# dsforza96/yocto-hair

Measured on AMD Instinct MI355X. Metric: Msamples/sec (whole node), 720x720x1536spp sphere-hairblock; per-pixel L2 vs CPU ref, higher is better.
Workload: dtype f32

## Files before the change

### include/yhair.h

```cpp
#ifndef YHAIR_H_
#define YHAIR_H_

#include <stdint.h>

#ifdef __cplusplus
extern "C" {
#endif

#define YH_OK 0
#define YH_E_INVALID -1
#define YH_E_DEVICE -2
#define YH_E_STATE -3
#define YH_E_IO -4
#define YH_E_SELFTEST -5


typedef struct yh_shape {
  int          num_vertices;
  const float* positions;
  const float* normals;
  const float* radius;
  int          num_lines;
  const int*   lines;
  int          num_triangles;
// ... 296 lines not shown
int yh_bvh_build_wide(int n, const float* boxes, int width, float* slots);

int yh_bvh_build_gpu(yh_context* ctx, int n, const float* boxes, float* nodes, int* primitives);
int yh_bvh_build_wide_gpu(yh_context* ctx, int n, const float* boxes, int width, float* slots);
int yh_bvh_refit_wide(int n, const float* boxes, const int* primitives, int width, float* slots);
int yh_bvh_refit_wide_gpu(yh_context* ctx, int n, const float* boxes, const int* primitives, int width, float* slots);

int yh_surface_lobe_batch(yh_context* ctx, int kind, int n, const float* params,
    const float* normal, const float* outgoing, const float* incoming,
    const float* rn, float* out);
int yh_surface_bsdf_batch(yh_context* ctx, int n, const yh_material* materials,
    const float* normal, const float* outgoing, const float* incoming,
    const float* rn, float* out);
int yh_intersect_batch(yh_context* ctx, int n, const float* rays, int* object,
    int* element, float* uv, float* distance);
#define YH_INTERSECT_FORMS 7
#define YH_INTERSECT_TABLE_IN_MEMORY 16
int yh_intersect_plain_batch(yh_context* ctx, int form, int n, const float* rays,
    int* object, int* element, float* uv, float* distance);
int yh_intersect_plain_form(int form);
int yh_scene_once(const yh_context* ctx);
int yh_lights_const_env(const yh_context* ctx);
int yh_shade_regions(const yh_context* ctx, uint64_t* out, int capacity);

int yh_lights_batch(yh_context* ctx, int form, int n, const float* position,
    const float* direction, const float* rn, float* out);

#define YH_VOLUME_FLOATS 24
int yh_volume_batch(yh_context* ctx, int form, int tex, int n,
    const yh_material* materials, const float* normal, const float* outgoing,
    const float* incoming, const float* texval, const float* rn, float* out);
#define YH_POINT_POSITION        0
#define YH_POINT_NORMAL          3
#define YH_POINT_SHADING_NORMAL  6
#define YH_POINT_TEXCOORD        9
#define YH_POINT_COLOR_TEX      11
#define YH_POINT_EMISSION_TEX   14
#define YH_POINT_EMISSION_TEX_X 17
#define YH_POINT_SCATTERING_TEX 18
#define YH_POINT_EMISSION       21
#define YH_POINT_BSDF           24
#define YH_POINT_DENSITY        46
#define YH_POINT_SCATTER        49
#define YH_POINT_ANISOTROPY     52
#define YH_POINT_FLOATS         53
int yh_point_batch(yh_context* ctx, int form, int n, const int* object,
// ... 34 lines not shown
```

### yocto-hair_amd/csrc/dev_items.h

```cpp
#ifndef YH_DEV_ITEMS_H_
#define YH_DEV_ITEMS_H_
#include "dev_path.h"

using namespace yhd;

#define YH_BLOCK 512
#define YH_MIN_WAVES 4

#define YH_QUADS (YH_BLOCK / 4)
template <bool COUNT, bool GENERAL, int BLOCK, int SHADER, int MODE = YH_MODE_QUAD, bool ONCE = false, bool TRIM = false, bool CENV = false>
YH_DEV void trace_items(const yhd_scene& sc, const yhd_state& st, int nsamples, yhd_counters* counters, unsigned int block = blockIdx.x,
    unsigned int blocks = gridDim.x) {
  constexpr int LPP    = YH_IS_HEX(MODE) ? 16 : YH_IS_OCT(MODE) ? 8 : 4;
  constexpr int GROUPS = BLOCK / LPP;
  extern __shared__ v4f lds_dyn[];
  YH_LDS unsigned int* lds_stack = (YH_LDS unsigned int*)lds_dyn;
  YH_LDS v4f*          lds_tabs  = (YH_LDS v4f*)(lds_stack + ((MODE == YH_MODE_QUAD ? sc.stack_entries : YH_IS_HEX(MODE) ? sc.stack_entries16 : sc.stack_entries8) + YH_HITROWS) * GROUPS);
  trace_ctx tc;
  tc.sc = &sc;
  tc.ls = nullptr, tc.sc_dev = nullptr;
  YH_LDS float* lds_cam;
  stage_tables(sc, lds_tabs, threadIdx.x, blockDim.x, tc, lds_cam);
  __syncthreads();

// ... 73 lines not shown
      }
      if (COUNT) {
        c1 = clock64(), cyc_trace += c1 - c0;
        unsigned int smax = steps;
        for (int off = 32; off > 0; off >>= 1) smax = max(smax, (unsigned int)__shfl_xor((int)smax, off, 64));
        w_steps += smax, l_steps += (lane & 3) == 0 ? steps : 0;
      }
      YH_REGION_MARK("shade_head");
      if (alive) {
        if constexpr (CENV) alive = path_step<COUNT, GROUPS, GENERAL, TRIM, CENV>(tc, ps, isec, rng, st.bounces, &ce);
        else if constexpr (SHADER == YH_SHADER_PATH) alive = path_step<COUNT, GROUPS, GENERAL, TRIM>(tc, ps, isec, rng, st.bounces);
        else alive = shade_step<COUNT, GROUPS, SHADER>(tc, ps, isec, rng, st.bounces);
        if (!alive) {
          YH_REGION_MARK("end");
          if (COUNT) stats.from = clock64();
          path_end(ps, st.clamp, acc);
          if (COUNT) count_quad<COUNT>(stats.samples);
          count_region<COUNT>(tc.stats, YH_REGION_END, stats.from);
        }
      }
      YH_REGION_MARK("loop_tail");
      if (COUNT) cyc_shade += clock64() - c1;
    }
    if (COUNT) {
      unsigned int v[11] = {stats.samples, stats.rays, stats.nodes, stats.seg, stats.tri, stats.hair, stats.surf,
          stats.envl, stats.envs, l_steps, l_iters};
      for (int k = 0; k < 11; k++)
        for (int off = 32; off > 0; off >>= 1) v[k] += (unsigned int)__shfl_xor((int)v[k], off, 64);
      if (lane == 0) {
        atomicAdd(&counters->samples, (unsigned long long)v[0]), atomicAdd(&counters->rays, (unsigned long long)v[1]);
        atomicAdd(&counters->nodes, (unsigned long long)v[2]), atomicAdd(&counters->seg, (unsigned long long)v[3]);
        atomicAdd(&counters->tri, (unsigned long long)v[4]), atomicAdd(&counters->hair, (unsigned long long)v[5]);
        atomicAdd(&counters->surf, (unsigned long long)v[6]), atomicAdd(&counters->envl, (unsigned long long)v[7]);
        atomicAdd(&counters->envs, (unsigned long long)v[8]);
        atomicAdd(&counters->lane_steps, (unsigned long long)v[9]), atomicAdd(&counters->lane_iters, (unsigned long long)v[10]);
        atomicAdd(&counters->cyc_trace, cyc_trace), atomicAdd(&counters->cyc_shade, cyc_shade);
        atomicAdd(&counters->wave_iters, (unsigned long long)w_iters), atomicAdd(&counters->wave_steps, (unsigned long long)w_steps);
      }
      if (lane == 0) {
        atomicAdd(&counters->c_geom, stats.c_geom), atomicAdd(&counters->c_sample, stats.c_sample);
        atomicAdd(&counters->c_eval, stats.c_eval), atomicAdd(&counters->c_rest, stats.c_rest);
      }
      {
        unsigned int b[10] = {stats.t_node, stats.l_node, stats.t_line, stats.l_line, stats.t_tri, stats.l_tri, stats.t_enter,
            stats.l_enter, stats.t_scene, stats.l_scene};
        for (int k = 0; k < 10; k++) {
          for (int off = 32; off > 0; off >>= 1) b[k] += (unsigned int)__shfl_xor((int)b[k], off, 64);
          if (lane == 0) atomicAdd(&counters->branch[k], (unsigned long long)b[k]);
        }
      }
      unsigned long long* sums = stats.r;
      if (lane < 3 * YH_REGIONS) atomicAdd(&counters->region[lane], sums[lane]), sums[lane] = 0;
      stats = stats_t{};
      stats.r = sums;
    }
    if (owner && (lane & (LPP - 1)) == 0) {
      st.rng_state[pix] = rng.state;
      st.accum[pix]     = acc;
    }
    if (lane == 0) {
      unsigned int dt = (unsigned int)(wall_clock64() - t0);
      if (YH_IS_OCT(MODE) || YH_IS_HEX(MODE)) atomicAdd(&st.tile_cost[item], dt);
      else st.tile_cost[item] = dt;
      if (COUNT) atomicAdd(&counters->cyc_tile, (unsigned long long)dt);
    }
  }
}
#define YH_OCT_BLOCK 256
template <bool COUNT, bool GENERAL, int BLOCK, int WAVES, int MODE = YH_MODE_QUAD, bool ONCE = false>
__global__ __launch_bounds__(BLOCK, WAVES) void k_trace(const yhd_scene sc, const yhd_state st,
    int nsamples, yhd_counters* counters) {
  static_assert(!ONCE || !GENERAL, "the prologue form exists for the plain variants");
  constexpr bool TRIM = !GENERAL && BLOCK == YH_BLOCK && MODE == YH_MODE_QUAD;
  trace_items<COUNT, GENERAL, BLOCK, YH_SHADER_PATH, MODE, ONCE, TRIM>(sc, st, nsamples, counters);
}
template <bool COUNT, bool ONCE>
__global__ __launch_bounds__(YH_BLOCK, YH_MIN_WAVES) void k_trace_cenv(const yhd_scene sc, const yhd_state st, int nsamples, yhd_counters* counters) {
  trace_items<COUNT, false, YH_BLOCK, YH_SHADER_PATH, YH_MODE_QUAD, ONCE, true, true>(sc, st, nsamples, counters);
}
template <bool GENERAL, bool ONCE = false>
__global__ __launch_bounds__(YH_BLOCK, YH_MIN_WAVES) void k_trace_sbs(const yhd_scene sc, const yhd_state st, int nsamples, int oct_blocks,
    int quad_items, int oct_entries) {
  if ((int)blockIdx.x < oct_blocks) {
    yhd_state so   = st;
    so.tiles       = st.tiles + quad_items, so.num_tiles = oct_entries, so.tile_cursor = st.tile_cursor + 16;
    trace_items<false, GENERAL, YH_BLOCK, YH_SHADER_PATH, YH_MODE_OCT, ONCE, !GENERAL>(sc, so, nsamples, nullptr, blockIdx.x, (unsigned)oct_blocks);
  } else {
// ... 20 lines not shown
```

### yocto-hair_amd/csrc/dev_trace.h

```cpp
#ifndef YH_DEV_TRACE_H_
#define YH_DEV_TRACE_H_
#include "dev_math.h"

namespace yhd {

struct rng_t {
  uint64_t state, inc;
};
YH_DEV uint32_t advance_rng(rng_t& rng) {
  uint64_t old        = rng.state;
  rng.state           = old * 6364136223846793005ULL + rng.inc;
  uint32_t xorshifted = (uint32_t)(((old >> 18u) ^ old) >> 27u);
  uint32_t rot        = (uint32_t)(old >> 59u);
  return (xorshifted >> rot) | (xorshifted << ((-rot) & 31));
}
YH_DEV float rand1f(rng_t& rng) {
  return __uint_as_float((advance_rng(rng) >> 9) | 0x3f800000u) - 1.0f;
}
YH_DEV rng_t make_rng(uint64_t seed, uint64_t seq) {
  rng_t rng;
  rng.state = 0U;
  rng.inc   = (seq << 1u) | 1u;
  advance_rng(rng);
  rng.state += seed;
  advance_rng(rng);
  return rng;
}

struct ray_t {
  f3    o, d;
  float tmin, tmax;
};
YH_DEV ray_t mkray(f3 o, f3 d) { return ray_t{o, d, ray_eps, flt_max}; }

struct hit_t {
  int   object, slot;
  float u, v, distance;
};

template <bool STRAIGHT = false, bool RAW = false>
YH_DEV bool intersect_line(f3 ro, f3 rd, float tmin, float tmax, f3 p0, f3 p1, float r0,
    float r1, float& uu, float& vv, float& dist, float a_in = 0.0f, float* rr = nullptr) {
  f3    u = rd, v = p1 - p0, w = ro - p0;
  float a = RAW ? a_in : dot(u, u), b = dot(u, v), c = dot(v, v), d = dot(u, w), e = dot(v, w);
  float det = a * c - b * b;
  if (STRAIGHT) {
    float t   = (b * e - c * d) / det;
    float s   = (a * e - b * d) / det;
    bool  ok  = det != 0 && !(t < tmin || t > tmax);
    s         = fclamp(s, 0.0f, 1.0f);
    f3    pr  = ro + rd * t;
    f3    pl  = p0 + (p1 - p0) * s;
    f3    prl = pr - pl;
    float d2  = dot(prl, prl);
    float r   = r0 * (1 - s) + r1 * s;
    ok        = ok && !(d2 > r * r);
    if (RAW) {
      uu = s, vv = d2, *rr = r, dist = t;
      return ok;
    }
    if (ok) uu = s, vv = sqrtf(d2) / r, dist = t;
    return ok;
  }
  if (det == 0) return false;
  float t = (b * e - c * d) / det;
  float s = (a * e - b * d) / det;
  if (t < tmin || t > tmax) return false;
  s        = fclamp(s, 0.0f, 1.0f);
// ... 6 lines not shown
  if (RAW) uu = s, vv = d2, *rr = r;
  else uu = s, vv = sqrtf(d2) / r;
  dist = t;
  return true;
}
YH_DEV bool intersect_triangle(f3 ro, f3 rd, float tmin, float tmax, f3 p0, f3 p1, f3 p2,
    float& uu, float& vv, float& dist) {
  f3    edge1 = p1 - p0, edge2 = p2 - p0;
  f3    pvec = cross(rd, edge2);
  float det  = dot(edge1, pvec);
  if (det == 0) return false;
  float inv_det = 1.0f / det;
  f3    tvec    = ro - p0;
  float u       = dot(tvec, pvec) * inv_det;
  if (u < 0 || u > 1) return false;
  f3    qvec = cross(tvec, edge1);
  float v    = dot(rd, qvec) * inv_det;
  if (v < 0 || u + v > 1) return false;
  float t = dot(edge2, qvec) * inv_det;
  if (t < tmin || t > tmax) return false;
  uu = u, vv = v;
  dist = t;
  return true;
}
YH_DEV bool intersect_bbox(f3 ro, f3 dinv, float tmin_, float tmax_, f3 bmin, f3 bmax) {
  f3    it_min = (bmin - ro) * dinv;
  f3    it_max = (bmax - ro) * dinv;
  f3    tmin   = {fmin_(it_min.x, it_max.x), fmin_(it_min.y, it_max.y), fmin_(it_min.z, it_max.z)};
  f3    tmax   = {fmax_(it_min.x, it_max.x), fmax_(it_min.y, it_max.y), fmax_(it_min.z, it_max.z)};
  float t0     = fmax_(hmax(tmin), tmin_);
  float t1     = fmin_(hmin(tmax), tmax_);
  t1 *= 1.00000024f;
  return t0 <= t1;
}

YH_DEV bool intersect_bbox_nonan(f3 ro, f3 dinv, float tmin_, float tmax_, f3 bmin, f3 bmax) {
  f3    it_min = (bmin - ro) * dinv;
  f3    it_max = (bmax - ro) * dinv;
  float t0 = __builtin_fmaxf(__builtin_fmaxf(__builtin_fminf(it_min.x, it_max.x), __builtin_fminf(it_min.y, it_max.y)),
      __builtin_fmaxf(__builtin_fminf(it_min.z, it_max.z), tmin_));
  float t1 = __builtin_fminf(__builtin_fminf(__builtin_fmaxf(it_min.x, it_max.x), __builtin_fmaxf(it_min.y, it_max.y)),
      __builtin_fminf(__builtin_fmaxf(it_min.z, it_max.z), tmax_));
  t1 *= 1.00000024f;
  return t0 <= t1;
}

// ... 139 lines not shown
  auto box_test = [](f3 o, f3 dinv, float t0, float t1, f3 bmin, f3 bmax) {
    return EXACT ? intersect_bbox(o, dinv, t0, t1, bmin, bmax) : intersect_bbox_nonan(o, dinv, t0, t1, bmin, bmax);
  };
  if (!EXACT && !wnonan) {
    redo = true;
    return hit;
  }
  f3    lo = ray.o, ld = ray.d, ldinv = wdinv;
  constexpr bool HOIST_A = STRIDE != 64;
  float ld2 = 0.0f;
  int   lsign = wsign | (wsign << 4), cur_obj = -1, kind = 0, node_base = 0;
  unsigned long long n_nodes = 0, n_seg = 0, n_tri = 0;
  unsigned int       n_steps = 0;

  const bool in_lds = LDS_SCENE || tc.lds_scene != nullptr;
  const bool wide_scene = !LDS_SCENE && sc.scene_wide_root >= 0;
  const YH_LDS v4f* lds_snodes = in_lds ? tc.lds_scene + YH_OBJECT_F4 * sc.num_objects : nullptr;
  auto scene_prim = [&](int i) -> int {
    if (in_lds) return ((const YH_LDS int*)(lds_snodes + 2 * sc.num_scene_nodes))[i];
    return sc.scene_prims[i];
  };
  static_assert(!ONCE || (LDS_SCENE && !EXACT), "the prologue form reads the scene level from LDS and leaves NaN slabs to the second pass");
  unsigned int cur;
  if constexpr (ONCE) {
    cur = YH_NONE;
    const v4f n0 = lds_snodes[0], n1 = lds_snodes[1];
    if (q == 0) n_nodes++;
    if (COUNT) count_branch<COUNT>(tc.stats->t_scene, tc.stats->l_scene);
    if (COUNT) count_branch<COUNT>(tc.stats->t_enter, tc.stats->l_enter);
    if (box_test(ray.o, wdinv, ray.tmin, tmax, xyz(n0), xyz(n1))) {
      const int start = __float_as_int(n0.w), num = __float_as_int(n1.w) & 0xffff;
      for (int k = num - 1; k >= 0; k--) {
        const int         obj = scene_prim(start + k);
        const YH_LDS v4f* ob  = tc.lds_scene + YH_OBJECT_F4 * obj;
        const f3    it_min = (xyz(ob[8]) - ray.o) * wdinv, it_max = (xyz(ob[9]) - ray.o) * wdinv;
        const float t0  = __builtin_fmaxf(__builtin_fmaxf(__builtin_fminf(it_min.x, it_max.x), __builtin_fminf(it_min.y, it_max.y)),
            __builtin_fmaxf(__builtin_fminf(it_min.z, it_max.z), ray.tmin));
        const float far = __builtin_fminf(__builtin_fminf(__builtin_fmaxf(it_min.x, it_max.x), __builtin_fmaxf(it_min.y, it_max.y)),
            __builtin_fmaxf(it_min.z, it_max.z));
        if (!(t0 <= __builtin_fminf(far, tmax) * 1.00000024f)) continue;
        const v4f a = ob[3], b = ob[4], c = ob[5];
        frame     inv;
        inv.x = {a.x, a.y, a.z}, inv.y = {a.w, b.x, b.y}, inv.z = {b.z, b.w, c.x}, inv.o = {c.y, c.z, c.w};
        const f3  o_ = transform_point(inv, ray.o), d_ = transform_vector(inv, ray.d), di = quad_rcp(d_);
        const int sg = (di.x < 0 ? 1 : 0) | (di.y < 0 ? 2 : 0) | (di.z < 0 ? 4 : 0);
        if (!(finite3(di) && finite3(o_))) redo = true;
        const int root = __float_as_int(YH_IS_HEX(MODE) ? ob[10].w : YH_IS_OCT(MODE) ? ob[10].z : ob[10].x);
        YH_LDS v4f* rec = tc.lds_once + 4 * k * STRIDE;
        rec[0]          = v4f{o_.x, o_.y, o_.z, t0};
        rec[STRIDE]     = v4f{d_.x, d_.y, d_.z, far};
        rec[2 * STRIDE] = v4f{di.x, di.y, di.z, dot(d_, d_)};
        rec[3 * STRIDE] = v4f{__int_as_float(sg), ob[6].x, __int_as_float(root), __int_as_float(obj)};
        if (cur != YH_NONE) push(cur);
        cur = YH_TAG_ENTER | (unsigned)k;
      }
    }
    if (redo) cur = YH_NONE, sp = 0;
  } else if (first_object >= 0) {
    cur = YH_TAG_ENTER | (unsigned)first_object;
  } else {
    if (sc.num_scene_nodes == 0) return hit;
    cur = YH_TAG_SCENE | 0u;
  }
  while (true) {
    if (COUNT) n_steps++;
    if (cur == YH_NONE) {
      if (sp == 0) break;
      cur = pop();
    }
    unsigned int tag = cur & YH_TAG_MASK;
    bool scene_node = false;
    if constexpr (ONCE) {
      if (tag == YH_TAG_ENTER) {
        if (COUNT) count_branch<COUNT>(tc.stats->t_enter, tc.stats->l_enter);
        const YH_LDS v4f* rec;
        v4f               r0, r1;
        while (true) {
          rec = tc.lds_once + 4 * (int)(cur & 3u) * STRIDE;
          r0 = rec[0], r1 = rec[STRIDE];
          if (r0.w <= __builtin_fminf(r1.w, tmax) * 1.00000024f) break;
          cur = YH_NONE;
          if (sp == 0) break;
          cur = pop();
        }
        if (cur == YH_NONE) continue;
        const v4f r2 = rec[2 * STRIDE], r3 = rec[3 * STRIDE];
        lo = xyz(r0), ld = xyz(r1), ldinv = xyz(r2), ld2 = r2.w;
        lsign = __float_as_int(r3.x), kind = __float_as_int(r3.y), node_base = __float_as_int(r3.z), cur_obj = __float_as_int(r3.w);
        cur = YH_TAG_SHAPE | (unsigned)node_base;
        tag = YH_TAG_SHAPE;
      }
    } else {
    if (!LDS_SCENE && tag == YH_TAG_SCENE && wide_scene) {
      if (COUNT) count_branch<COUNT>(tc.stats->t_scene, tc.stats->l_scene);
      const unsigned int low = cur & ~YH_TAG_MASK;
      if (low >= (1u << 27)) {
        const int start = (int)(low & 0x07FFFFFFu), num = (int)(low >> 27);
        if ((int)q >= 1 && (int)q < num) YH_STK(sp + (num - 1 - (int)q)) = YH_TAG_ENTER | (unsigned)sc.scene_prims[start + (int)q];
        sp += num - 1;
        cur = YH_TAG_ENTER | (unsigned)sc.scene_prims[start];
        tag = YH_TAG_ENTER;
      } else {
        scene_node = true;
        lo = ray.o, ldinv = wdinv, lsign = (lsign & 0x70) | (lsign >> 4);
        cur = low;
        tag = YH_TAG_SHAPE;
      }
    } else if (tag == YH_TAG_SCENE) {
      if (COUNT) count_branch<COUNT>(tc.stats->t_scene, tc.stats->l_scene);
      int idx = (int)(cur & ~YH_TAG_MASK);
      v4f n0, n1;
      if (in_lds) n0 = lds_snodes[2 * idx], n1 = lds_snodes[2 * idx + 1];
      else n0 = ldg4(sc.scene_nodes + 2 * idx), n1 = ldg4(sc.scene_nodes + 2 * idx + 1);
      if (q == 0) n_nodes++;
      cur = YH_NONE;
// ... 35 lines not shown
      if (in_lds) {
        const YH_LDS v4f* ob = tc.lds_scene + YH_OBJECT_F4 * cur_obj;
        v4f a = ob[3], b = ob[4], c = ob[5], d = ob[6];
        inv.x = {a.x, a.y, a.z}, inv.y = {a.w, b.x, b.y}, inv.z = {b.z, b.w, c.x}, inv.o = {c.y, c.z, c.w};
        kind = __float_as_int(d.x);
        node_base = __float_as_int(YH_IS_HEX(MODE) ? ob[10].w : YH_IS_OCT(MODE) ? ob[10].z : ob[10].x);
      } else {
        const yhd_object& o = sc.objects[cur_obj];
        inv       = ldframe(o.inv_frame);
        kind      = o.kind;
        node_base = YH_IS_HEX(MODE) ? o.lane_root16 : YH_IS_OCT(MODE) ? o.lane_root8 : o.lane_root;
      }
      lo    = transform_point(inv, ray.o);
      ld    = transform_vector(inv, ray.d);
      ldinv = quad_rcp(ld);
      lsign = (lsign & 0x70) | (ldinv.x < 0 ? 1 : 0) | (ldinv.y < 0 ? 2 : 0) | (ldinv.z < 0 ? 4 : 0);
      if (!EXACT && !(finite3(ldinv) && finite3(lo))) {
        redo = true;
        break;
      }
      if (HOIST_A) ld2 = dot(ld, ld);
      cur = YH_TAG_SHAPE | (unsigned)node_base;
      tag = YH_TAG_SHAPE;
    }
    }
    {
      bool is_leaf    = tag == YH_TAG_LEAF;
      constexpr bool     GROUPS = MODE == YH_MODE_OCTP || MODE == YH_MODE_HEXP;
      const unsigned int qj     = MODE == YH_MODE_HEXP ? (__lane_id() >> 2) & 3u : MODE == YH_MODE_OCTP ? (__lane_id() >> 2) & 1u : 0u;
      int                grp    = 0;
      bool               idle   = false;
      unsigned int       mycur  = cur;
      if (GROUPS) {
        const bool   look = is_leaf && qj > 0 && sp >= (int)qj;
        unsigned int pk   = look ? YH_STK(sp - (int)qj) : 0u;
        unsigned int lb   = (look && (pk & YH_TAG_MASK) == YH_TAG_LEAF) ? (1u << qj) : 0u;
        lb |= (unsigned int)dpp_i<YH_ROW_HALF_MIRROR>((int)lb);
        if (MODE == YH_MODE_HEXP) lb |= (unsigned int)dpp_i<YH_ROW_MIRROR>((int)lb);
        grp   = (lb & 2u) ? ((lb & 4u) ? ((lb & 8u) ? 3 : 2) : 1) : 0;
        idle  = is_leaf && (int)qj > grp;
        mycur = (qj > 0 && !idle) ? pk : cur;
      }
      int  leaf_start = (int)(mycur & 0x07FFFFFFu), leaf_num = (int)((mycur >> 27) & 7u);
      bool mine       = !is_leaf || (int)q < leaf_num;
      int  pq         = mine ? (int)q : leaf_num - 1;
      const unsigned int nslot = (MODE == YH_MODE_QUAD || scene_node) ? q : (__lane_id() & (YH_IS_HEX(MODE) ? 15u : 7u));
      const yhd_float4*  addr  = sc.lane_blob + 2 * (size_t)(is_leaf ? (unsigned)leaf_start + (unsigned)pq * (kind == YH_KIND_LINES ? 1u : 2u) : cur + nslot);
// ... 181 lines not shown
```

### yocto-hair_amd/csrc/yh_device.h

```cpp
#ifndef YH_DEVICE_H_
#define YH_DEVICE_H_
#include <stdint.h>

#define YH_KIND_LINES 1
#define YH_KIND_TRIANGLES 2
#define YH_TILE 8
#define YH_MAX_LIGHTS 16
#define YH_MAX_ENVS 4

typedef struct yhd_float4 { float x, y, z, w; } yhd_float4;
typedef struct yhd_int4 { int x, y, z, w; } yhd_int4;

typedef struct yhd_object {
  float frame[12];
  float inv_frame[12];
  int   kind;
  int   node_base;
  int   prim_base;
  int   vert_base;
  int   elem_base;
  int   has_normals;
  int   material;
  int   has_texcoords;
  float wbox_min[4], wbox_max[4];
// ... 176 lines not shown
  yhd_int4   own;
} yhd_path_slot;
typedef struct yhd_stream {
  yhd_path_slot* slots;
  yhd_float4* medium;
  unsigned int* stack_ovf;
  unsigned long long* prof;
  unsigned long long* wave_log;
  const int*  wave_begin;
  int*        wave_fill;
  int         slots_per_wave;
  int         ovf_entries;
  long long   total_slots;
  int         prof_parts_only;
  int         suspend_lanes;
} yhd_stream;

typedef struct yhd_counters {
  unsigned long long samples, rays, nodes, seg, tri, hair, surf, envl, envs;
  unsigned long long cyc_trace, cyc_shade, cyc_tile, wave_iters, wave_steps, lane_steps, lane_iters;
  unsigned long long c_geom, c_sample, c_eval, c_rest;
  unsigned long long branch[10];
  unsigned long long region[3 * 9];
} yhd_counters;
enum yhd_region {
  YH_REGION_REGEN = 0,
  YH_REGION_MISS,
  YH_REGION_FETCH,
  YH_REGION_HAIR,
  YH_REGION_SAMPLE,
  YH_REGION_EVAL,
  YH_REGION_LIGHTS_PDF,
  YH_REGION_WEIGHT,
  YH_REGION_END,
  YH_REGIONS
};
static_assert(YH_REGIONS == 9, "yhd_counters::region");

#endif
```

### yocto-hair_amd/host/context_internal.h

```cpp
#ifndef YH_CONTEXT_INTERNAL_H_
#define YH_CONTEXT_INTERNAL_H_
#include <hip/hip_runtime_api.h>
#include <dlfcn.h>
#include <fcntl.h>
#include <sys/stat.h>
#include <unistd.h>
#include <rccl/rccl.h>

#include <algorithm>
#include <chrono>
#include <cmath>
#include <cstdarg>
#include <cstddef>
#include <cstdio>
#include <cstdlib>
#include <cstring>
#include <limits>
#include <map>
#include <mutex>
#include <tuple>
#include <string>
#include <memory>
#include <thread>
#include <vector>
// ... 102 lines not shown
  std::vector<yhd_maps>         h_dmaps;
  bool                          big_lights = false;
  bool                          light_edits = false;
  DevBuf                        d_env_cdf[YH_MAX_ENVS];
  yh_camera                     key_camera{};
  std::vector<unsigned char>    key_geometry, key_envs;
  std::vector<yhh::Box>         h_shape_roots, h_obj_boxes;
  DevBuf                        d_shape_roots;
  int                           max_shape_depth = 0, max_shape_depth8 = 0, max_shape_depth16 = 0;
  int                           scene_wide_room = 0;
  struct ShapeState {
    int    num_vertices, has_normals, has_texcoords, per_vertex, vert_base, elem_base, depth, depth8, depth16, count[3], room[3];
    size_t key_positions;
    int    wide_levels[3], wide_first[3][66];
    double area_build[3], area_now[3];
  };
  std::vector<ShapeState>       shape_states;
  bool             have_state = false;
  yhd_state        state{};
  yh_trace_params  params{};
  DevBuf           d_textures, d_tex_texels, d_vtex, d_maps;
  DevBuf           d_rng_state, d_rng_inc, d_accum, d_tiles, d_image, d_counters, d_tile_cursor, d_tile_cost, d_display;
  unsigned long long last_regions[3 * YH_REGIONS] = {};
  std::vector<int> owned;
  std::vector<unsigned int>  item_cost;
  int              rank = 0, world = 1;
  int              num_tiles_total = 0;
  float            last_ms = 0;
  int              last_launches = 0;
  float            dn_ms[1 + YH_DENOISE_MAX_ITERATIONS] = {};
  int              dn_ms_count = 0;
  struct Temporal {
    bool             have = false, have_moments = false;
    int              width = 0, height = 0, side = 0, num_objects = 0;
    DevBuf           hc[2], hg[2], hm[2], d_var, d_frames, d_usable;
    yh_camera        camera{};
    std::vector<int> usable;
  } tp;
  int              last_nsamples = 0;
  unsigned         launches_of_image = 0;
  int              launch_shape = YH_SHAPE_QUAD;
  int              last_shape = -1;
  bool             async_pending = false;
  bool             last_counted = false;
  DevBuf                  d_gather_send, d_gather_recv;
  std::vector<ncclComm_t> comms;
// ... 136 lines not shown
```

### yocto-hair_amd/host/trace_launch.cpp

```cpp
#include "context_internal.h"

int wait_for_launch(yh_context* ctx) {
  if (ctx->poisoned) return refuse_poisoned(ctx);
  const double timeout = yhh::launch_timeout_s();
  const int    device  = ctx->device;
  hipStream_t  stream  = ctx->stream;
  int          e       = 0;
  const double spin_s  = std::min(std::min(0.050, timeout), 1.25e-3 * (double)ctx->last_ms + 0.001);
  {
    const auto t0 = std::chrono::steady_clock::now();
    while (true) {
      const hipError_t q = hipStreamQuery(stream);
      if (q == hipSuccess) return YH_OK;
      if (q != hipErrorNotReady) return fail(ctx, YH_E_DEVICE, "hipStreamQuery: %s", hipGetErrorString(q));
      if (std::chrono::duration<double>(std::chrono::steady_clock::now() - t0).count() > spin_s) break;
    }
  }
  const int    rc      = ctx->sync_call.run(
      [device, stream]() {
        hipError_t se = hipSetDevice(device);
        return (int)(se != hipSuccess ? se : hipStreamSynchronize(stream));
      },
      timeout, &e);
  if (rc == yhh::WAIT_EXPIRED) {
// ... 262 lines not shown
}
int yh_launch_shape(const yh_context* ctx) { return ctx ? ctx->last_shape : YH_E_INVALID; }
int yh_kernel_trials(const yh_context* ctx, double* ms_per_sample, int* trials, int count) {
  if (!ctx || !ms_per_sample || !trials || count < 1) return YH_E_INVALID;
  for (int k = 0; k < count; k++) {
    ms_per_sample[k] = k < YH_SHAPES ? ctx->shape_ms[k] : 0.0;
    trials[k]        = k < YH_SHAPES ? ctx->shape_trials[k] : 0;
    if (std::isinf(ms_per_sample[k])) ms_per_sample[k] = -1.0;
  }
  return YH_SHAPES;
}
int yh_trials_pending(const yh_context* ctx) { return ctx ? (trial_pending(ctx) ? 1 : 0) : YH_E_INVALID; }
int yh_last_trace_ms(const yh_context* ctx, float* ms, int* launches) {
  if (!ctx) return YH_E_INVALID;
  if (ms) *ms = ctx->last_ms;
  if (launches) *launches = ctx->last_launches;
  return YH_OK;
}
int yh_trace_samples_counted(yh_context* ctx, int nsamples, yh_workcounts* out) {
  if (!ctx || !out) return YH_E_INVALID;
  if (!ctx->have_state) return fail(ctx, YH_E_STATE, "yh_trace_samples_counted before yh_init_state");
  HIPCHK(ctx, hipSetDevice(ctx->device));
  HIPCHK(ctx, hipMemsetAsync(ctx->d_counters.p, 0, sizeof(yhd_counters), ctx->stream));
  int rc = trace_impl(ctx, nsamples, true, true);
  if (rc) return rc;
  yhd_counters c;
  HIPCHK(ctx, hipMemcpy(&c, ctx->d_counters.p, sizeof(c), hipMemcpyDeviceToHost));
  out->samples = c.samples, out->rays = c.rays, out->nodes = c.nodes, out->seg_tests = c.seg, out->tri_tests = c.tri;
  out->hair_shades = c.hair, out->surf_shades = c.surf, out->env_lookups = c.envl, out->env_samples = c.envs;
  out->cyc_trace = c.cyc_trace, out->cyc_shade = c.cyc_shade, out->ticks_tile = c.cyc_tile, out->wave_iters = c.wave_iters;
  out->wave_steps = c.wave_steps, out->lane_steps = c.lane_steps, out->lane_iters = c.lane_iters;
  out->cyc_geom = c.c_geom, out->cyc_sample = c.c_sample, out->cyc_eval = c.c_eval, out->cyc_rest = c.c_rest;
  for (int k = 0; k < 10; k++) out->branch[k] = c.branch[k];
  for (int k = 0; k < 3 * YH_REGIONS; k++) ctx->last_regions[k] = c.region[k];
  return YH_OK;
}
int yh_shade_regions(const yh_context* ctx, uint64_t* out, int capacity) {
  if (!ctx || !out || capacity < 0) return YH_E_INVALID;
  for (int k = 0; k < capacity && k < 3 * YH_REGIONS; k++) out[k] = ctx->last_regions[k];
  return 3 * YH_REGIONS;
}
```

### yocto-hair_amd/python/yhair_capi.py

```python
import ctypes as C
import os

import numpy as np

ROOT = os.path.dirname(os.path.dirname(os.path.dirname(os.path.abspath(__file__))))
LIB_PATH = os.environ.get("YHAIR_LIB", os.path.join(ROOT, "yocto-hair_amd", "libyhair.so"))

YH_OK, YH_E_INVALID, YH_E_DEVICE, YH_E_STATE, YH_E_IO, YH_E_SELFTEST = 0, -1, -2, -3, -4, -5
YH_HAIR_BRDF_FLOATS = 30
HAIR_SHADE_FLOATS = 15
SURFACE_BSDF_FLOATS = 29
VOLUME_FLOATS = 24
QUAD_FORMS_FLOATS = 12
PATH_BEGIN, PATH_CONTINUE, PATH_END = 0, 1, 2
PATH_OPS = {"begin": PATH_BEGIN, "continue": PATH_CONTINUE, "end": PATH_END}
PATH_ROWS = {PATH_BEGIN: (17, 4, 12, 3), PATH_CONTINUE: (3, 2, 3, 2), PATH_END: (8, 1, 4, 0)}
INTERSECT_FORMS = 7
INTERSECT_TABLE_IN_MEMORY = 16
POINT_FLOATS = 53
POINT_COLUMNS = {"position": slice(0, 3), "normal": slice(3, 6), "shading_normal": slice(6, 9), "texcoord": slice(9, 11),
                 "color_tex": slice(11, 14), "emission_tex": slice(14, 17), "emission_tex_x": slice(17, 18),
                 "scattering_tex": slice(18, 21), "emission": slice(21, 24), "bsdf": slice(24, 46), "density": slice(46, 49),
                 "scatter": slice(49, 52), "anisotropy": slice(52, 53)}
(LOBE_DIFFUSE, LOBE_SPECULAR, LOBE_METAL, LOBE_TRANSMISSION, LOBE_REFRACTION, LOBE_DELTA_SPECULAR,
# ... 259 lines not shown
                                     c_float_p, c_float_p, c_int_p]),
    "yh_bvh_build_gpu": (C.c_int, [C.c_void_p, C.c_int, c_float_p, c_float_p, c_int_p]),
    "yh_bvh_build": (C.c_int, [C.c_int, c_float_p, c_float_p, c_int_p]),
    "yh_bvh_build_wide": (C.c_int, [C.c_int, c_float_p, C.c_int, c_float_p]),
    "yh_bvh_build_wide_gpu": (C.c_int, [C.c_void_p, C.c_int, c_float_p, C.c_int, c_float_p]),
    "yh_bvh_refit_wide": (C.c_int, [C.c_int, c_float_p, c_int_p, C.c_int, c_float_p]),
    "yh_bvh_refit_wide_gpu": (C.c_int, [C.c_void_p, C.c_int, c_float_p, c_int_p, C.c_int, c_float_p]),
    "yh_surface_lobe_batch": (C.c_int, [C.c_void_p, C.c_int, C.c_int, c_float_p, c_float_p, c_float_p, c_float_p,
                                        c_float_p, c_float_p]),
    "yh_surface_bsdf_batch": (C.c_int, [C.c_void_p, C.c_int, C.POINTER(Material), c_float_p, c_float_p, c_float_p,
                                        c_float_p, c_float_p]),
    "yh_hair_eval_batch": (C.c_int, [C.c_void_p, C.c_int, c_float_p, c_float_p, c_float_p, c_float_p]),
    "yh_hair_sample_batch": (C.c_int, [C.c_void_p, C.c_int, c_float_p, c_float_p, c_float_p, c_float_p]),
    "yh_hair_pdf_batch": (C.c_int, [C.c_void_p, C.c_int, c_float_p, c_float_p, c_float_p, c_float_p]),
    "yh_hair_eval_pdf_batch": (C.c_int, [C.c_void_p, C.c_int, c_float_p, c_float_p, c_float_p, c_float_p]),
    "yh_hair_shade_batch": (C.c_int, [C.c_void_p, C.c_int, C.c_int, C.c_int, C.POINTER(Material), c_float_p, c_float_p, c_float_p,
                                      c_float_p, c_float_p, c_float_p, c_float_p]),
    "yh_intersect_batch": (C.c_int, [C.c_void_p, C.c_int, c_float_p, c_int_p, c_int_p, c_float_p, c_float_p]),
    "yh_intersect_plain_batch": (C.c_int, [C.c_void_p, C.c_int, C.c_int, c_float_p, c_int_p, c_int_p, c_float_p, c_float_p]),
    "yh_intersect_plain_form": (C.c_int, [C.c_int]),
    "yh_scene_once": (C.c_int, [C.c_void_p]),
    "yh_lights_const_env": (C.c_int, [C.c_void_p]),
    "yh_shade_regions": (C.c_int, [C.c_void_p, C.POINTER(C.c_uint64), C.c_int]),
    "yh_lights_batch": (C.c_int, [C.c_void_p, C.c_int, C.c_int, c_float_p, c_float_p, c_float_p, c_float_p]),
    "yh_volume_batch": (C.c_int, [C.c_void_p, C.c_int, C.c_int, C.c_int, C.POINTER(Material), c_float_p, c_float_p, c_float_p, c_float_p,
                                  c_float_p, c_float_p]),
    "yh_point_batch": (C.c_int, [C.c_void_p, C.c_int, C.c_int, c_int_p, c_int_p, c_float_p, c_float_p, c_float_p]),
    "yh_quad_forms_batch": (C.c_int, [C.c_void_p, C.c_int, c_float_p, c_float_p, c_float_p, c_float_p, c_float_p]),
    "yh_path_ends_batch": (C.c_int, [C.c_void_p, C.c_int, C.c_int, C.c_int, c_float_p, c_int_p, C.POINTER(C.c_uint64), c_float_p, c_int_p,
                                     C.POINTER(C.c_uint64)]),
    "yh_selftest": (C.c_int, [C.c_void_p, C.c_int, c_float_p]),
    "yh_scene_load": (C.c_void_p, [C.c_char_p, C.c_char_p, C.c_char_p, C.c_int]),
    "yh_scene_get": (C.POINTER(SceneDesc), [C.c_void_p]),
    "yh_scene_get_maps": (C.POINTER(MaterialMaps), [C.c_void_p]),
    "yh_scene_free": (None, [C.c_void_p]),
    "yh_save_image": (C.c_int, [C.c_char_p, C.c_int, C.c_int, c_float_p, C.c_char_p, C.c_int]),
}
EXPORTS = tuple(_SIGS)

_lib = None


def load(path=None):
    global _lib
    if _lib is None or path:
        p = path or LIB_PATH
# ... 811 lines not shown
        uv, dist = np.zeros((n, 2), np.float32), np.zeros(n, np.float32)
        self._chk(self.lib.yh_intersect_plain_batch(self.h, form, n, fptr(rays), iptr(obj), iptr(elem), fptr(uv), fptr(dist)))
        return obj, elem, uv, dist

    def scene_once(self):
        rc = int(self.lib.yh_scene_once(self.h))
        if rc < 0:
            self._chk(rc)
        return rc

    def lights_const_env(self):
        rc = int(self.lib.yh_lights_const_env(self.h))
        if rc < 0:
            self._chk(rc)
        return rc

    SHADE_REGIONS = ("regen", "miss", "fetch", "hair", "sample", "eval", "lights_pdf", "weight", "end")

    def shade_regions(self):
        out = (C.c_uint64 * 27)()
        self.lib.yh_shade_regions(self.h, out, 27)
        return {nm: (int(out[3 * k]), int(out[3 * k + 1]), int(out[3 * k + 2])) for k, nm in enumerate(self.SHADE_REGIONS)}

    def lights(self, form, position, direction, rn4):
        a = [np.ascontiguousarray(x, np.float32) for x in (position, direction, rn4)]
        n = len(a[0])
        out = np.zeros((n, 8), np.float32)
        self._chk(self.lib.yh_lights_batch(self.h, form, n, *(fptr(x) for x in a), fptr(out)))
        return out

    def selftest(self, which):
        worst = C.c_float()
        rc = self.lib.yh_selftest(self.h, which, C.byref(worst))
        if rc not in (YH_OK, YH_E_SELFTEST):
            self._chk(rc)
        return rc == YH_OK, worst.value
```

Baseline: 2738.

## Add dedicated once-per-ray traversal loop with flattened object entries and one-return intersectors

```diff
diff --git a/include/yhair.h b/include/yhair.h
--- a/include/yhair.h
+++ b/include/yhair.h
@@ -342,6 +342,7 @@
 int yh_scene_once(const yh_context* ctx);
 int yh_lights_const_env(const yh_context* ctx);
 int yh_shade_regions(const yh_context* ctx, uint64_t* out, int capacity);
+int yh_set_count_bound(yh_context* ctx, int items);
 
 int yh_lights_batch(yh_context* ctx, int form, int n, const float* position,
     const float* direction, const float* rn, float* out);
diff --git a/yocto-hair_amd/csrc/dev_items.h b/yocto-hair_amd/csrc/dev_items.h
--- a/yocto-hair_amd/csrc/dev_items.h
+++ b/yocto-hair_amd/csrc/dev_items.h
@@ -119,12 +119,13 @@
       YH_REGION_MARK("loop_tail");
       if (COUNT) cyc_shade += clock64() - c1;
     }
+    const bool item_counted = COUNT && (counters->counted_items == nullptr || counters->counted_items[item] != 0);
     if (COUNT) {
       unsigned int v[11] = {stats.samples, stats.rays, stats.nodes, stats.seg, stats.tri, stats.hair, stats.surf,
           stats.envl, stats.envs, l_steps, l_iters};
       for (int k = 0; k < 11; k++)
         for (int off = 32; off > 0; off >>= 1) v[k] += (unsigned int)__shfl_xor((int)v[k], off, 64);
-      if (lane == 0) {
+      if (lane == 0 && item_counted) {
         atomicAdd(&counters->samples, (unsigned long long)v[0]), atomicAdd(&counters->rays, (unsigned long long)v[1]);
         atomicAdd(&counters->nodes, (unsigned long long)v[2]), atomicAdd(&counters->seg, (unsigned long long)v[3]);
         atomicAdd(&counters->tri, (unsigned long long)v[4]), atomicAdd(&counters->hair, (unsigned long long)v[5]);
@@ -134,7 +135,7 @@
         atomicAdd(&counters->cyc_trace, cyc_trace), atomicAdd(&counters->cyc_shade, cyc_shade);
         atomicAdd(&counters->wave_iters, (unsigned long long)w_iters), atomicAdd(&counters->wave_steps, (unsigned long long)w_steps);
       }
-      if (lane == 0) {
+      if (lane == 0 && item_counted) {
         atomicAdd(&counters->c_geom, stats.c_geom), atomicAdd(&counters->c_sample, stats.c_sample);
         atomicAdd(&counters->c_eval, stats.c_eval), atomicAdd(&counters->c_rest, stats.c_rest);
       }
@@ -143,11 +144,14 @@
             stats.l_enter, stats.t_scene, stats.l_scene};
         for (int k = 0; k < 10; k++) {
           for (int off = 32; off > 0; off >>= 1) b[k] += (unsigned int)__shfl_xor((int)b[k], off, 64);
-          if (lane == 0) atomicAdd(&counters->branch[k], (unsigned long long)b[k]);
+          if (lane == 0 && item_counted) atomicAdd(&counters->branch[k], (unsigned long long)b[k]);
         }
       }
       unsigned long long* sums = stats.r;
-      if (lane < 3 * YH_REGIONS) atomicAdd(&counters->region[lane], sums[lane]), sums[lane] = 0;
+      if (lane < 3 * YH_REGIONS) {
+        if (item_counted) atomicAdd(&counters->region[lane], sums[lane]);
+        sums[lane] = 0;
+      }
       stats = stats_t{};
       stats.r = sums;
     }
@@ -159,7 +163,7 @@
       unsigned int dt = (unsigned int)(wall_clock64() - t0);
       if (YH_IS_OCT(MODE) || YH_IS_HEX(MODE)) atomicAdd(&st.tile_cost[item], dt);
       else st.tile_cost[item] = dt;
-      if (COUNT) atomicAdd(&counters->cyc_tile, (unsigned long long)dt);
+      if (COUNT && item_counted) atomicAdd(&counters->cyc_tile, (unsigned long long)dt);
     }
   }
 }
diff --git a/yocto-hair_amd/csrc/dev_trace.h b/yocto-hair_amd/csrc/dev_trace.h
--- a/yocto-hair_amd/csrc/dev_trace.h
+++ b/yocto-hair_amd/csrc/dev_trace.h
@@ -38,12 +38,26 @@
   float u, v, distance;
 };
 
-template <bool STRAIGHT = false, bool RAW = false>
+template <bool STRAIGHT = false, bool RAW = false, bool ONE_RETURN = false>
 YH_DEV bool intersect_line(f3 ro, f3 rd, float tmin, float tmax, f3 p0, f3 p1, float r0,
     float r1, float& uu, float& vv, float& dist, float a_in = 0.0f, float* rr = nullptr) {
   f3    u = rd, v = p1 - p0, w = ro - p0;
   float a = RAW ? a_in : dot(u, u), b = dot(u, v), c = dot(v, v), d = dot(u, w), e = dot(v, w);
   float det = a * c - b * b;
+  if (ONE_RETURN) {
+    static_assert(!ONE_RETURN || RAW, "the one-return form hands out the raw results");
+    float t = (b * e - c * d) / det;
+    float s = (a * e - b * d) / det;
+    if (!(det != 0 && !(t < tmin || t > tmax))) return false;
+    s         = fclamp(s, 0.0f, 1.0f);
+    f3    pr  = ro + rd * t;
+    f3    pl  = p0 + (p1 - p0) * s;
+    f3    prl = pr - pl;
+    float d2  = dot(prl, prl);
+    float r   = r0 * (1 - s) + r1 * s;
+    uu = s, vv = d2, *rr = r, dist = t;
+    return !(d2 > r * r);
+  }
   if (STRAIGHT) {
     float t   = (b * e - c * d) / det;
     float s   = (a * e - b * d) / det;
@@ -96,6 +110,20 @@
   uu = u, vv = v;
   dist = t;
   return true;
+}
+YH_DEV bool intersect_triangle_one_return(f3 ro, f3 rd, float tmin, float tmax, f3 p0, f3 p1, f3 p2, float& uu, float& vv, float& dist) {
+  f3    edge1 = p1 - p0, edge2 = p2 - p0;
+  f3    pvec = cross(rd, edge2);
+  float det  = dot(edge1, pvec);
+  float inv_det = 1.0f / det;
+  f3    tvec    = ro - p0;
+  float u       = dot(tvec, pvec) * inv_det;
+  if (!(det != 0 && !(u < 0 || u > 1))) return false;
+  f3    qvec = cross(tvec, edge1);
+  float v    = dot(rd, qvec) * inv_det;
+  float t    = dot(edge2, qvec) * inv_det;
+  uu = u, vv = v, dist = t;
+  return !(v < 0 || u + v > 1) && !(t < tmin || t > tmax);
 }
 YH_DEV bool intersect_bbox(f3 ro, f3 dinv, float tmin_, float tmax_, f3 bmin, f3 bmax) {
   f3    it_min = (bmin - ro) * dinv;
@@ -281,6 +309,7 @@
   };
   static_assert(!ONCE || (LDS_SCENE && !EXACT), "the prologue form reads the scene level from LDS and leaves NaN slabs to the second pass");
   unsigned int cur;
+  int          ent = 0;
   if constexpr (ONCE) {
     cur = YH_NONE;
     const v4f n0 = lds_snodes[0], n1 = lds_snodes[1];
@@ -305,22 +334,136 @@
         const int sg = (di.x < 0 ? 1 : 0) | (di.y < 0 ? 2 : 0) | (di.z < 0 ? 4 : 0);
         if (!(finite3(di) && finite3(o_))) redo = true;
         const int root = __float_as_int(YH_IS_HEX(MODE) ? ob[10].w : YH_IS_OCT(MODE) ? ob[10].z : ob[10].x);
-        YH_LDS v4f* rec = tc.lds_once + 4 * k * STRIDE;
+        YH_LDS v4f* rec = tc.lds_once + 4 * ent * STRIDE;
         rec[0]          = v4f{o_.x, o_.y, o_.z, t0};
         rec[STRIDE]     = v4f{d_.x, d_.y, d_.z, far};
         rec[2 * STRIDE] = v4f{di.x, di.y, di.z, dot(d_, d_)};
         rec[3 * STRIDE] = v4f{__int_as_float(sg), ob[6].x, __int_as_float(root), __int_as_float(obj)};
-        if (cur != YH_NONE) push(cur);
-        cur = YH_TAG_ENTER | (unsigned)k;
-      }
-    }
-    if (redo) cur = YH_NONE, sp = 0;
+        ent++;
+        lo = o_, ld = d_, ldinv = di, ld2 = dot(d_, d_);
+        lsign = sg, kind = __float_as_int(ob[6].x), node_base = root, cur_obj = obj;
+      }
+    }
+    if (ent > 0) ent--, cur = YH_TAG_SHAPE | (unsigned)node_base;
+    if (redo) ent = 0, cur = YH_NONE;
   } else if (first_object >= 0) {
     cur = YH_TAG_ENTER | (unsigned)first_object;
   } else {
     if (sc.num_scene_nodes == 0) return hit;
     cur = YH_TAG_SCENE | 0u;
   }
+  if constexpr (ONCE) {
+    static_assert(MODE == YH_MODE_QUAD || MODE == YH_MODE_OCT, "the once-per-ray form exists for quads and octets");
+    hrec[3 * STRIDE] = YH_NONE;
+    if (cur != YH_NONE) do {
+      if (COUNT) n_steps++;
+      const bool         is_leaf = (cur & YH_TAG_MASK) == YH_TAG_LEAF;
+      const bool         lines   = kind == YH_KIND_LINES;
+      const unsigned int leaf_start = cur & 0x07FFFFFFu, leaf_num = (cur >> 27) & 7u;
+      const bool         mine  = q < leaf_num;
+      const unsigned int pq    = mine ? q : leaf_num - 1u;
+      const unsigned int nslot = MODE == YH_MODE_QUAD ? q : (__lane_id() & 7u);
+      const unsigned int unit = is_leaf ? leaf_start + (lines ? pq : 2u * pq) : cur + nslot;
+      const yhd_float4*  addr = sc.lane_blob + 2 * (size_t)unit;
+      const v4f          s0 = ldg4(addr), s1 = ldg4(addr + 1);
+      auto leaf_end = [&](bool ok, float uu, float vv, float dist, float rr) {
+        const int my_i  = (int)q;
+        int       key_i = ok ? my_i : -1;
+        float     key_t = ok ? dist : __builtin_inff();
+#define YH_KEY_MERGE(CTRL)                                                   \
+  {                                                                         \
+    int   oi = dpp_i<CTRL>(key_i);                                          \
+    float ot = dpp_f<CTRL>(key_t);                                          \
+    bool  take = (ot < key_t) | ((ot == key_t) & (oi > key_i));             \
+    key_i = take ? oi : key_i, key_t = take ? ot : key_t;                   \
+  }
+        YH_KEY_MERGE(YH_QUAD_XOR1)
+        YH_KEY_MERGE(YH_QUAD_XOR2)
+#undef YH_KEY_MERGE
+        tmax = key_i >= 0 ? key_t : tmax;
+        if (key_i == my_i) {
+          hrec[0] = __float_as_uint(uu), hrec[STRIDE] = __float_as_uint(vv), hrec[2 * STRIDE] = __float_as_uint(rr);
+          hrec[3 * STRIDE] = ((unsigned)cur_obj << 28) | (leaf_start + (lines ? q : 2u * q));
+        }
+        cur = YH_NONE;
+      };
+      if (!is_leaf) {
+        if (q == 0) n_nodes++;
+        if (COUNT) count_branch<COUNT>(tc.stats->t_node, tc.stats->l_node);
+        const unsigned int ref  = __float_as_uint(s1.z);
+        const unsigned int axes = __float_as_uint(s1.w);
+        const bool h = intersect_bbox_nonan(lo, ldinv, ray.tmin, tmax, f3{s0.x, s0.y, s0.z}, f3{s0.w, s1.x, s1.y}) && ref != YH_NONE;
+        unsigned int rank, M;
+        if (MODE == YH_MODE_QUAD) {
+          const unsigned int pair = q >> 1;
+          const unsigned int sgn  = (lsign >> ((axes >> (2 + 2 * pair)) & 3)) & 1;
+          const unsigned int s0_  = (lsign >> (axes & 3)) & 1;
+          rank = ((pair ^ s0_) << 1) | ((q & 1) ^ sgn);
+        } else {
+          const unsigned int g  = (__lane_id() & 7u) >> 1;
+          const unsigned int n0 = (lsign >> (axes & 3)) & 1;
+          const unsigned int n1 = (lsign >> ((axes >> (2 + 2 * (g >> 1))) & 3)) & 1;
+          const unsigned int n2 = (lsign >> ((axes >> (6 + 2 * g)) & 3)) & 1;
+          rank = ((((g >> 1) ^ n0) << 2) | (((g & 1) ^ n1) << 1)) | ((__lane_id() & 1u) ^ n2);
+        }
+        const unsigned int bit = h ? (1u << rank) : 0u;
+        M = bit | (unsigned int)dpp_i<YH_QUAD_XOR1>((int)bit);
+        M |= (unsigned int)dpp_i<YH_QUAD_XOR2>((int)M);
+        if (MODE == YH_MODE_OCT) M |= (unsigned int)dpp_i<YH_ROW_HALF_MIRROR>((int)M);
+        const bool first = h && (M & (bit - 1)) == 0;
+        if (h && !first) YH_STK(sp + (int)__popc(M >> (rank + 1))) = ref;
+        unsigned int head = first ? ref : 0u;
+        head |= (unsigned int)dpp_i<YH_QUAD_XOR1>((int)head);
+        head |= (unsigned int)dpp_i<YH_QUAD_XOR2>((int)head);
+        if (MODE == YH_MODE_OCT) head |= (unsigned int)dpp_i<YH_ROW_HALF_MIRROR>((int)head);
+        const int nh = __popc(M);
+        sp += nh > 0 ? nh - 1 : 0;
+        cur = nh > 0 ? head : YH_NONE;
+      }
+      if (is_leaf) {
+        if (lines) {
+          if (COUNT) count_branch<COUNT>(tc.stats->t_line, tc.stats->l_line);
+          float uu, vv, dist, rr;
+          if (mine) n_seg++;
+          const bool ok = intersect_line<(STRIDE == 64), true, (STRIDE != 64)>(lo, ld, ray.tmin, tmax, xyz(s0), xyz(s1), s0.w, s1.w, uu, vv, dist, HOIST_A ? ld2 : dot(ld, ld), &rr);
+          leaf_end(ok & mine, uu, vv, dist, rr);
+        } else {
+          if (COUNT) count_branch<COUNT>(tc.stats->t_tri, tc.stats->l_tri);
+          const v4f s2 = ldg4(addr + 2);
+          float     uu, vv, dist;
+          if (mine) n_tri++;
+          const bool ok = intersect_triangle_one_return(lo, ld, ray.tmin, tmax, xyz(s0), xyz(s1), xyz(s2), uu, vv, dist);
+          leaf_end(ok & mine, uu, vv, dist, 1.0f);
+        }
+      }
+      if (cur == YH_NONE) {
+        if (sp > 0) {
+          cur = pop();
+        } else if (ent > 0) {
+          if (COUNT) count_branch<COUNT>(tc.stats->t_enter, tc.stats->l_enter);
+          int take = -1;
+#pragma unroll
+          for (int s = 0; s < 3; s++) {
+            if (s + 1 >= sc.scene_once) break;
+            const YH_LDS float* w  = (const YH_LDS float*)(tc.lds_once + 4 * s * STRIDE);
+            const float         t0 = w[3], far = w[4 * STRIDE + 3];
+            const bool          in = (s < ent) & (t0 <= __builtin_fminf(far, tmax) * 1.00000024f);
+            take = in ? s : take;
+          }
+          ent = take < 0 ? 0 : take;
+          if (take >= 0) {
+            const YH_LDS v4f* rec = tc.lds_once + 4 * take * STRIDE;
+            const v4f         r0 = rec[0], r1 = rec[STRIDE], r2 = rec[2 * STRIDE], r3 = rec[3 * STRIDE];
+            lo = xyz(r0), ld = xyz(r1), ldinv = xyz(r2), ld2 = r2.w;
+            lsign = __float_as_int(r3.x), kind = __float_as_int(r3.y), node_base = __float_as_int(r3.z), cur_obj = __float_as_int(r3.w);
+            cur = YH_TAG_SHAPE | (unsigned)node_base;
+          }
+        }
+      }
+    } while (cur != YH_NONE);
+    const unsigned int packed = hrec[3 * STRIDE];
+    if (packed != YH_NONE) hit.object = (int)(packed >> 28), hit.slot = (int)(packed & 0x0FFFFFFFu), hit.distance = tmax;
+  } else
   while (true) {
     if (COUNT) n_steps++;
     if (cur == YH_NONE) {
@@ -329,27 +472,6 @@
     }
     unsigned int tag = cur & YH_TAG_MASK;
     bool scene_node = false;
-    if constexpr (ONCE) {
-      if (tag == YH_TAG_ENTER) {
-        if (COUNT) count_branch<COUNT>(tc.stats->t_enter, tc.stats->l_enter);
-        const YH_LDS v4f* rec;
-        v4f               r0, r1;
-        while (true) {
-          rec = tc.lds_once + 4 * (int)(cur & 3u) * STRIDE;
-          r0 = rec[0], r1 = rec[STRIDE];
-          if (r0.w <= __builtin_fminf(r1.w, tmax) * 1.00000024f) break;
-          cur = YH_NONE;
-          if (sp == 0) break;
-          cur = pop();
-        }
-        if (cur == YH_NONE) continue;
-        const v4f r2 = rec[2 * STRIDE], r3 = rec[3 * STRIDE];
-        lo = xyz(r0), ld = xyz(r1), ldinv = xyz(r2), ld2 = r2.w;
-        lsign = __float_as_int(r3.x), kind = __float_as_int(r3.y), node_base = __float_as_int(r3.z), cur_obj = __float_as_int(r3.w);
-        cur = YH_TAG_SHAPE | (unsigned)node_base;
-        tag = YH_TAG_SHAPE;
-      }
-    } else {
     if (!LDS_SCENE && tag == YH_TAG_SCENE && wide_scene) {
       if (COUNT) count_branch<COUNT>(tc.stats->t_scene, tc.stats->l_scene);
       const unsigned int low = cur & ~YH_TAG_MASK;
@@ -431,7 +553,6 @@
       if (HOIST_A) ld2 = dot(ld, ld);
       cur = YH_TAG_SHAPE | (unsigned)node_base;
       tag = YH_TAG_SHAPE;
-    }
     }
     {
       bool is_leaf    = tag == YH_TAG_LEAF;
diff --git a/yocto-hair_amd/csrc/yh_device.h b/yocto-hair_amd/csrc/yh_device.h
--- a/yocto-hair_amd/csrc/yh_device.h
+++ b/yocto-hair_amd/csrc/yh_device.h
@@ -222,6 +222,7 @@
   unsigned long long c_geom, c_sample, c_eval, c_rest;
   unsigned long long branch[10];
   unsigned long long region[3 * 9];
+  const unsigned char* counted_items;
 } yhd_counters;
 enum yhd_region {
   YH_REGION_REGEN = 0,
diff --git a/yocto-hair_amd/host/context_internal.h b/yocto-hair_amd/host/context_internal.h
--- a/yocto-hair_amd/host/context_internal.h
+++ b/yocto-hair_amd/host/context_internal.h
@@ -148,6 +148,8 @@
   DevBuf           d_textures, d_tex_texels, d_vtex, d_maps;
   DevBuf           d_rng_state, d_rng_inc, d_accum, d_tiles, d_image, d_counters, d_tile_cursor, d_tile_cost, d_display;
   unsigned long long last_regions[3 * YH_REGIONS] = {};
+  int              count_bound = 0;
+  DevBuf           d_counted_items;
   std::vector<int> owned;
   std::vector<unsigned int>  item_cost;
   int              rank = 0, world = 1;
diff --git a/yocto-hair_amd/host/trace_launch.cpp b/yocto-hair_amd/host/trace_launch.cpp
--- a/yocto-hair_amd/host/trace_launch.cpp
+++ b/yocto-hair_amd/host/trace_launch.cpp
@@ -308,6 +308,16 @@
   if (!ctx->have_state) return fail(ctx, YH_E_STATE, "yh_trace_samples_counted before yh_init_state");
   HIPCHK(ctx, hipSetDevice(ctx->device));
   HIPCHK(ctx, hipMemsetAsync(ctx->d_counters.p, 0, sizeof(yhd_counters), ctx->stream));
+  if (ctx->count_bound > 0) {
+    std::vector<int> items;
+    build_work_items(ctx, items);
+    std::vector<unsigned char> counted(ctx->item_cost.size(), 0);
+    for (size_t k = 0; k < items.size() && k < (size_t)ctx->count_bound; k++) counted[(size_t)items[k]] = 1;
+    if (int urc = upload_keep(ctx, ctx->d_counted_items, counted.data(), counted.size())) return urc;
+    const unsigned char* flags = (const unsigned char*)ctx->d_counted_items.p;
+    HIPCHK(ctx, hipMemcpyAsync((char*)ctx->d_counters.p + offsetof(yhd_counters, counted_items), &flags, sizeof(flags), hipMemcpyHostToDevice, ctx->stream));
+    YH_WAIT(ctx);
+  }
   int rc = trace_impl(ctx, nsamples, true, true);
   if (rc) return rc;
   yhd_counters c;
@@ -321,6 +331,11 @@
   for (int k = 0; k < 3 * YH_REGIONS; k++) ctx->last_regions[k] = c.region[k];
   return YH_OK;
 }
+int yh_set_count_bound(yh_context* ctx, int items) {
+  if (!ctx || items < 0) return YH_E_INVALID;
+  ctx->count_bound = items;
+  return YH_OK;
+}
 int yh_shade_regions(const yh_context* ctx, uint64_t* out, int capacity) {
   if (!ctx || !out || capacity < 0) return YH_E_INVALID;
   for (int k = 0; k < capacity && k < 3 * YH_REGIONS; k++) out[k] = ctx->last_regions[k];
diff --git a/yocto-hair_amd/python/yhair_capi.py b/yocto-hair_amd/python/yhair_capi.py
--- a/yocto-hair_amd/python/yhair_capi.py
+++ b/yocto-hair_amd/python/yhair_capi.py
@@ -305,6 +305,7 @@
     "yh_scene_once": (C.c_int, [C.c_void_p]),
     "yh_lights_const_env": (C.c_int, [C.c_void_p]),
     "yh_shade_regions": (C.c_int, [C.c_void_p, C.POINTER(C.c_uint64), C.c_int]),
+    "yh_set_count_bound": (C.c_int, [C.c_void_p, C.c_int]),
     "yh_lights_batch": (C.c_int, [C.c_void_p, C.c_int, C.c_int, c_float_p, c_float_p, c_float_p, c_float_p]),
     "yh_volume_batch": (C.c_int, [C.c_void_p, C.c_int, C.c_int, C.c_int, C.POINTER(Material), c_float_p, c_float_p, c_float_p, c_float_p,
                                   c_float_p, c_float_p]),
@@ -1162,6 +1163,9 @@
         self.lib.yh_shade_regions(self.h, out, 27)
         return {nm: (int(out[3 * k]), int(out[3 * k + 1]), int(out[3 * k + 2])) for k, nm in enumerate(self.SHADE_REGIONS)}
 
+    def set_count_bound(self, items):
+        self._chk(self.lib.yh_set_count_bound(self.h, int(items)))
+
     def lights(self, form, position, direction, rn4):
         a = [np.ascontiguousarray(x, np.float32) for x in (position, direction, rn4)]
         n = len(a[0])
```

Result: faster. 2977, median of 6 (+8.7%).
